# noir-lang/acvm

Hardware: AMD Instinct MI355X
Metric: witnesses solved/sec (whole node) (higher is better)
Workload: dtype u256 (8x u32 limbs, BN254-Fr Montgomery); 1 GPU; 10000-gate arithmetic-only ACIR, batch 2^20 witnesses over 1 GPU(s); opcodes=10000, global_batch=1048576, instances_per_gpu=1048576, tile_instances=131072, levels=41, not_solved_rank0_all_steps=68, algorithmic_bytes_per_witness=1025376, brillig_opcodes_inlined=0, parallelism=instances sharded x1, no collectives

## Files before the change

### acvm_amd/__init__.py

```python
import ctypes as C
import functools
import os

from . import acir

_HERE = os.path.dirname(os.path.abspath(__file__))
LIB_PATH = os.environ.get("ACVM_AMD_LIB") or os.path.join(_HERE, "libacvm_amd.so")

STATUS_SOLVED, STATUS_IN_PROGRESS, STATUS_FAILURE, STATUS_REQUIRES_FOREIGN_CALL = 0, 1, 2, 3
(ERR_NONE, ERR_MISSING_ASSIGNMENT, ERR_TOO_MANY_UNKNOWNS, ERR_UNSUPPORTED_BLACKBOX, ERR_UNSATISFIED, ERR_INDEX_OOB,
 ERR_BLACKBOX_FAILED, ERR_BRILLIG_FAILED, ERR_PANIC, ERR_DEVICE_LIMIT) = range(10)
LIMIT_BRILLIG_STEPS, LIMIT_BRILLIG_CALL_DEPTH, LIMIT_BRILLIG_MEMORY, LIMIT_DEVICE_MEMORY = 1, 2, 3, 4
ENC_BE32, ENC_LE32, ENC_MONT256_LE = 0, 1, 2
ENC_U8, ENC_U16, ENC_U32, ENC_U64, ENC_U128 = 16, 17, 18, 19, 20
LAYOUT_INSTANCE_MAJOR, LAYOUT_WITNESS_MAJOR = 0, 1
LAYOUT_BROADCAST = 16

ABI_SYMBOLS = [
    "acvm_last_error", "acvm_abi_version", "acvm_device_count", "acvm_set_device", "acvm_device_synchronize",
    "acvm_device_arch", "acvm_selftest", "acvm_debug_grumpkin", "acvm_debug_secp", "acvm_circuit_from_bytes", "acvm_circuit_free", "acvm_circuit_num_opcodes",
    "acvm_circuit_num_witnesses", "acvm_circuit_plan_stats", "acvm_batch_new", "acvm_batch_free", "acvm_batch_set_initial_witness",
    "acvm_batch_set_initial_witness_device", "acvm_batch_solve", "acvm_batch_solve_then_import", "acvm_batch_reset", "acvm_batch_set_instances", "acvm_batch_set_force_slow_path",
    "acvm_batch_results", "acvm_batch_witness", "acvm_batch_witness_map", "acvm_batch_stats",
    "acvm_batch_set_profiling", "acvm_batch_pending_foreign_call", "acvm_batch_pending_foreign_call_inputs",
    "acvm_batch_resolve_foreign_call", "acvm_circuit_assert_message", "acvm_circuit_witness_set", "acvm_batch_error_string",
    "acvm_batch_extract_witnesses", "acvm_batch_digest", "acvm_witness_map_decode", "acvm_witness_map_encode", "acvm_batch_witness_map_bytes",
    "acvm_device_malloc", "acvm_device_free", "acvm_device_upload", "acvm_batch_solve_opcode", "acvm_bb_stubbed", "acvm_bb_dummy",
    "acvm_new", "acvm_free", "acvm_solve", "acvm_solve_opcode", "acvm_get_status", "acvm_instruction_pointer", "acvm_witness_map", "acvm_finalize",
    "acvm_get_pending_foreign_call", "acvm_pending_foreign_call_inputs", "acvm_resolve_pending_foreign_call",
    "acvm_multi_new", "acvm_multi_free", "acvm_multi_num_groups", "acvm_multi_solve", "acvm_multi_results", "acvm_multi_num_witnesses",
    "acvm_multi_witness_map", "acvm_multi_locate", "acvm_debug_modmul_rate", "acvm_debug_secp_rate", "acvm_batch_new_ex", "acvm_circuit_plan_stats_ex",
    "acvm_tuning_set", "acvm_tuning_get", "acvm_tuning_key",
    "acvm_device_release_tables", "acvm_circuit_opcode_kinds", "acvm_batch_error_expression", "acvm_debug_stream_rate", "acvm_node_new", "acvm_node_free", "acvm_node_tile_instances", "acvm_node_num_devices", "acvm_node_solve", "acvm_node_stats",
    "acvm_debug_cpulist", "acvm_debug_device_locality", "acvm_debug_plan_fingerprint", "acvm_circuit_plans_built", "acvm_circuit_check_schedule", "acvm_batch_digest_blake2s",
    "acvm_batch_export_device", "acvm_device_download", "acvm_debug_fr", "acvm_debug_inverse_batch",
    "acvm_batch_import_device", "acvm_batch_solve_then_import_ex",
    "acvm_batch_import_device_parts", "acvm_debug_import_list_copies",
    "acvm_batch_import_device_masked", "acvm_batch_set_initial_witness_masked", "acvm_debug_import_missing",
    "acvm_debug_table_info", "acvm_debug_table_read", "acvm_debug_batch_tables",
    "acvm_batch_outcomes_device", "acvm_batch_export_device_list", "acvm_debug_export_h2d_bytes", "acvm_debug_select",
    "acvm_node_solve_device", "acvm_debug_node_io_bytes",
    "acvm_batch_foreign_call_sites", "acvm_batch_foreign_call_inputs_device", "acvm_batch_resolve_foreign_calls_device", "acvm_debug_foreign_call_stats",
    "acvm_batch_resolve_foreign_calls_device_rows",
    "acvm_node_set_foreign_call_handler", "acvm_node_foreign_stats",
    "acvm_batch_import_device_records", "acvm_batch_set_initial_witness_records", "acvm_node_solve_records",
    "acvm_batch_export_device_records", "acvm_batch_witness_records",
]


class AcvmError(RuntimeError):
    pass


class ExpressionHead(C.Structure):
    _fields_ = [("n_mul", C.c_uint32), ("n_lin", C.c_uint32), ("opcode_index", C.c_uint32), ("q_c", C.c_uint8 * 32)]


class ExportDesc(C.Structure):
# ... 364 lines not shown
    L.acvm_batch_results.argtypes = [C.c_void_p, C.c_void_p]
    L.acvm_batch_witness.argtypes = [C.c_void_p, C.c_uint32, C.c_void_p, C.c_void_p]
    L.acvm_batch_witness_map.argtypes = [C.c_void_p, C.c_uint32, C.c_uint32, C.c_void_p, C.c_void_p]
    L.acvm_batch_stats.argtypes = [C.c_void_p, C.POINTER(Stats)]
    L.acvm_batch_pending_foreign_call.argtypes = [C.c_void_p, C.c_uint32, C.POINTER(ForeignCallInfo)]
    L.acvm_batch_pending_foreign_call_inputs.argtypes = [C.c_void_p, C.c_uint32, C.c_void_p, C.c_void_p]
    L.acvm_batch_resolve_foreign_call.argtypes = [C.c_void_p, C.c_uint32, C.c_uint32, C.c_char_p, C.c_void_p, C.c_char_p]
    L.acvm_circuit_assert_message.argtypes = [C.c_void_p, C.c_uint32, C.c_uint32, C.c_char_p, C.c_size_t]
    L.acvm_circuit_witness_set.argtypes = [C.c_void_p, C.c_int, C.c_void_p, C.c_uint32]
    L.acvm_batch_error_string.argtypes = [C.c_void_p, C.c_void_p, C.c_uint32, C.c_char_p, C.c_size_t]
    L.acvm_batch_extract_witnesses.argtypes = [C.c_void_p, C.c_void_p, C.c_uint32, C.c_uint32, C.c_uint32, C.c_void_p]
    L.acvm_batch_digest.argtypes = [C.c_void_p, C.c_uint32, C.c_uint32, C.c_void_p]
    L.acvm_batch_digest_blake2s.argtypes = [C.c_void_p, C.c_uint32, C.c_uint32, C.c_void_p]
    for f in (L.acvm_witness_map_decode, L.acvm_witness_map_encode, L.acvm_batch_witness_map_bytes):
        f.restype = C.c_longlong
    L.acvm_witness_map_decode.argtypes = [C.c_char_p, C.c_size_t, C.c_void_p, C.c_void_p, C.c_uint32]
    L.acvm_witness_map_encode.argtypes = [C.c_void_p, C.c_char_p, C.c_uint32, C.c_void_p, C.c_size_t]
    L.acvm_batch_witness_map_bytes.argtypes = [C.c_void_p, C.c_uint32, C.c_void_p, C.c_size_t]
    L.acvm_debug_modmul_rate.argtypes = [C.c_uint32, C.c_uint32, C.POINTER(C.c_double), C.POINTER(C.c_uint64)]
    if hasattr(L, "acvm_debug_fr"):
        L.acvm_debug_fr.argtypes = [C.c_uint32, C.c_void_p, C.c_uint32, C.c_void_p, C.c_void_p]
        L.acvm_debug_inverse_batch.argtypes = [C.c_void_p, C.c_uint32, C.c_uint32, C.c_uint32, C.c_void_p, C.c_void_p, C.c_void_p, C.POINTER(C.c_uint32),
                                               C.POINTER(C.c_uint32)]
    L.acvm_debug_secp_rate.argtypes = [C.c_uint32, C.c_uint32, C.c_uint32, C.POINTER(C.c_double), C.POINTER(C.c_uint64)]
    L.acvm_circuit_opcode_kinds.argtypes = [C.c_void_p, C.c_uint32, C.c_uint32, C.c_void_p]
    L.acvm_batch_error_expression.argtypes = [C.c_void_p, C.c_void_p, C.c_uint32, C.POINTER(ExpressionHead), C.c_void_p, C.c_void_p, C.c_uint32, C.c_void_p, C.c_void_p, C.c_uint32]
    L.acvm_device_release_tables.restype = C.c_longlong
    L.acvm_device_release_tables.argtypes = [C.c_int]
    L.acvm_node_new.restype = C.c_void_p
    L.acvm_node_new.argtypes = [C.c_void_p, C.c_void_p, C.c_void_p, C.c_uint32, C.c_void_p, C.c_uint32, C.c_void_p]
    L.acvm_node_free.restype = None
    L.acvm_node_free.argtypes = [C.c_void_p]
    L.acvm_node_tile_instances.argtypes = [C.c_void_p]
    L.acvm_node_tile_instances.restype = C.c_uint32
    L.acvm_node_num_devices.argtypes = [C.c_void_p]
    L.acvm_node_num_devices.restype = C.c_uint32
    L.acvm_node_solve.restype = C.c_longlong
    L.acvm_node_solve.argtypes = [C.c_void_p, C.c_uint64, C.c_void_p, C.c_void_p, C.c_void_p, C.c_void_p, C.c_void_p]
    L.acvm_node_stats.argtypes = [C.c_void_p, C.c_void_p]
    L.acvm_debug_stream_rate.argtypes = [C.c_size_t, C.POINTER(C.c_double)]
    L.acvm_tuning_set.argtypes = [C.c_char_p, C.c_longlong]
    L.acvm_tuning_get.argtypes = [C.c_char_p, C.POINTER(C.c_longlong)]
    L.acvm_tuning_key.restype = C.c_char_p
    L.acvm_tuning_key.argtypes = [C.c_uint]
    L.acvm_device_malloc.restype = C.c_void_p
    L.acvm_device_malloc.argtypes = [C.c_size_t]
# ... 232 lines not shown
    assert all(len(it) == wi for it in items)
    data = b"".join(int(v).to_bytes(32, "big") for it in items for v in it)
    out = C.create_string_buffer(32 * wo * max(len(items), 1))
    _check(lib().acvm_debug_secp(curve, what, data, len(items), out))
    raw = out.raw
    return [tuple(int.from_bytes(raw[32 * (wo * i + k):32 * (wo * i + k + 1)], "big") for k in range(wo)) for i in range(len(items))]


FR_PROBE_WORDS = ((16, 8), (16, 8), (8, 8), (16, 8), (16, 8), (8, 8), (8, 8), (8, 8), (8, 8), (8, 2), (8, 2), (1, 8), (8, 9), (9, 8), (18, 9), (18, 9), (9, 9),
                  (9, 1), (9, 9), (10, 9), (9, 9), (9, 9), (9, 9), (9, 9), (19, 9), (18, 9), (9, 9), (9, 1), (18, 9), (36, 9), (54, 9), (27, 9), (45, 9), (27, 9),
                  (45, 9), (18, 9), (36, 9), (27, 9))


def debug_fr(what, items, uniform=None):
    import numpy as np
    wi, wo = FR_PROBE_WORDS[what]
    a = np.ascontiguousarray(items, dtype=np.uint32).reshape(-1, wi)
    out = np.zeros((a.shape[0], wo), dtype=np.uint32)
    u = None if uniform is None else np.ascontiguousarray(uniform, dtype=np.uint32).reshape(18)
    _check(lib().acvm_debug_fr(what, a.ctypes.data, a.shape[0], None if u is None else u.ctypes.data, out.ctypes.data))
    return out


def debug_inverse_batch(den, inv_chunk, slot_of=None):
    import numpy as np
    d = np.ascontiguousarray(den, dtype=np.uint32)
    n_jobs, B = d.shape[0], d.shape[1]
    assert d.shape == (n_jobs, B, 8)
    s = None if slot_of is None else np.ascontiguousarray(slot_of, dtype=np.uint32).reshape(n_jobs)
    inv, ev = np.zeros((n_jobs, B, 8), dtype=np.uint32), np.zeros(B, dtype=np.uint32)
    dc, hc = C.c_uint32(), C.c_uint32()
    _check(lib().acvm_debug_inverse_batch(d.ctypes.data, n_jobs, B, inv_chunk, None if s is None else s.ctypes.data, inv.ctypes.data, ev.ctypes.data,
                                          C.byref(dc), C.byref(hc)))
    return inv, ev, dc.value, hc.value


def debug_select(status, select_mask, out=None, want_list=True):
    import numpy as np
    st = np.ascontiguousarray(status, dtype=np.uint8).reshape(-1)
    n = st.shape[0]
    lst = None
    if want_list:
        lst = np.zeros(n, dtype=np.uint32) if out is None else np.ascontiguousarray(out, dtype=np.uint32).reshape(n).copy()
    count = C.c_uint32()
    _check(lib().acvm_debug_select(st.ctypes.data if n else None, n, select_mask, lst.ctypes.data if lst is not None and n else None, C.byref(count)))
    return lst, count.value


def decompress_witness(data: bytes) -> dict:
    n = _check(lib().acvm_witness_map_decode(data, len(data), None, None, 0))
    ids = (C.c_uint32 * max(n, 1))()
    vals = C.create_string_buffer(32 * max(n, 1))
    _check(lib().acvm_witness_map_decode(data, len(data), ids, vals, n))
    return {ids[i]: int.from_bytes(vals.raw[32 * i:32 * i + 32], "big") for i in range(n)}


# ... 722 lines not shown
```

### acvm_amd/csrc/batch_schedule.cpp

```cpp
#include <algorithm>
#include <chrono>
#include <cstdio>
#include <cstdlib>
#include <cstring>
#include <map>
#include <memory>
#include <new>
#include <stdexcept>
#include <string>
#include <vector>
#include "batch_internal.hpp"

struct LaunchTimers {
    std::vector<std::pair<hipEvent_t, hipEvent_t>> reg_pairs, dyn_pairs, cls_pairs[N_CLS];
    size_t ev_used = 0;
};

static int enqueue_level_schedule(acvm_batch *b, LaunchTimers *tm) {
    const Plan &p = b->plan();
    auto next_event = [&]() -> hipEvent_t {
        if (tm->ev_used == b->ev_pool.size()) {
            hipEvent_t e;
            hipEventCreate(&e);
            b->ev_pool.push_back(e);
// ... 19 lines not shown
            b->events_fresh = false;
            break;
        case SO_GATES:
            launch_arith_level(s, b->d_W, b->Bp, b->B, b->d_gate_stream, b->d_gate_offset + st.first, st.count, b->d_consts, b->d_event, b->d_inv);
            break;
        case SO_GATES_LIGHT:
            launch_arith_light_level(s, b->d_W, b->Bp, b->B, b->d_gate_stream, b->d_gate_offset + st.first, st.count, b->d_inv, b->dp,
                                     b->d_cls_offset[CLS_LIGHT] + st.first2, st.count2, b->d_event);
            break;
        case SO_LIGHT: launch_light_level(s, b->d_W, b->Bp, b->B, b->dp, off, st.count, b->d_event); break;
        case SO_LIGHT_SL: launch_light_sl_level(s, b->d_W, b->Bp, b->B, b->dp, off, st.count, b->d_event); break;
        case SO_HASH_COOP: launch_hash_coop_level(s, b->d_W, b->Bp, b->B, b->dp, off, st.count, b->d_event, st.lds_words); break;
        case SO_HASH: launch_hash_level(s, b->d_W, b->Bp, b->B, b->dp, off, soff, st.count, b->d_event, b->d_cls_scratch[k]); break;
        case SO_GRUMPKIN: launch_grumpkin_level(s, b->d_W, b->Bp, b->B, b->dp, off, soff, st.count, b->d_event, b->d_cls_scratch[k]); break;
        case SO_BRILLIG: launch_brillig_level(s, b->d_W, b->Bp, b->B, b->dp, off, soff, st.count, b->d_event, b->d_cls_scratch[k]); break;
        case SO_PEDERSEN: launch_pedersen_level(s, b->d_W, b->Bp, b->B, b->dp, off, st.count, b->d_event, soff, b->d_cls_scratch[k]); break;
        case SO_ECDSA: launch_ecdsa_level(s, b->d_W, b->Bp, b->B, b->dp, off, st.count, b->d_event); break;
        case SO_DIGEST: launch_digest_fold_level(s, b->d_W, b->Bp, b->B, b->dp, off, st.count, b->fp, b->d_leaves); break;
        case SO_HOSTBB:
            for (uint32_t r = 0; r < st.count; r++)
                if (int rc = run_host_blackbox(b, p.prog[p.cls_offset[k][st.first + r] + 1], false, 0)) return rc;
            break;
        case SO_INVERSE:
            launch_inverse_batch(s, b->d_W, b->d_inv, b->Bp, b->B, b->d_gate_stream, b->d_dyn_offset + st.first, st.count, b->d_event, (uint32_t)p.tune.inv_chunk);
            break;
        case SO_TRUNCATE: launch_event_truncate(s, b->d_event, b->B, p.truncated_at); break;
        }
        if (timed) {
            e1 = next_event();
            hipEventRecord(e1, s);
            (st.op == SO_GATES || st.op == SO_GATES_LIGHT ? tm->reg_pairs : st.op == SO_INVERSE ? tm->dyn_pairs : tm->cls_pairs[k]).push_back({e0, e1});
        }
        if (st.op == SO_GATES || st.op == SO_GATES_LIGHT) b->n_launches += (st.count + 65534) / 65535;
        else if (st.op != SO_EVENT_RESET && st.op != SO_TRUNCATE) b->n_launches++;
    }
    return 0;
}

static int ensure_level_events(acvm_batch *b) {
    const size_t n_levels = b->plan().n_levels;
    while (b->ev_sync.size() < 2 * n_levels + 1 || b->ev_heavy.size() < 4 * n_levels) {
        hipEvent_t e;
        HIPCHK(hipEventCreateWithFlags(&e, hipEventDisableTiming));
        (b->ev_sync.size() < 2 * n_levels + 1 ? b->ev_sync : b->ev_heavy).push_back(e);
    }
    return 0;
}
// ... 196 lines not shown
```

### acvm_amd/csrc/inverse_batch.hpp

```cpp
#pragma once
#include "fr_device.hpp"

namespace acvm {

template <class P>
FR_HD __forceinline__ void inverse_batch_body(const uint4 *__restrict__ W, uint4 *__restrict__ Inv, uint64_t Bp, uint64_t j, const uint32_t *__restrict__ gate_stream,
                                              const uint32_t *__restrict__ job_offset, uint32_t first, uint32_t n, uint32_t *__restrict__ event) {
    Fr29 prefix = fr29_from(fr_one());
    for (uint32_t i = 0; i < n; i++) {
        const uint32_t *__restrict__ g = gate_stream + job_offset[first + i];
        Fr den = P::load_den(W, g[0], Bp, j);
        if (fr_is_zero(den)) {
            P::flag(event, j, g[1]);
            den = fr_one();
        }
        prefix = fr29_mul(prefix, fr29_from(den));
        P::park(Inv, g[2], Bp, j, fr29_pack(prefix));
    }
    Fr29 inv = fr29_from(fr_inv(fr29_pack(fr29_cond_sub_p(prefix))));
    for (uint32_t i = n; i-- > 0;) {
        const uint32_t *__restrict__ g = gate_stream + job_offset[first + i];
        Fr den = P::load_den_last(W, g[0], Bp, j);
        if (fr_is_zero(den)) den = fr_one();
        const Fr prev = i > 0 ? P::parked(Inv, gate_stream[job_offset[first + i - 1] + 2], Bp, j) : fr_one();
        const Fr29 inv_i = fr29_mul(inv, fr29_from(prev));
        inv = fr29_mul(inv, fr29_from(den));
        P::store_inverse(Inv, g[2], Bp, j, fr29_pack(inv_i));
    }
}

}
```

### acvm_amd/csrc/kernels.hip

```cpp
#include "ops_common.hpp"
#include "fr_probe.hpp"
#include "inverse_batch.hpp"
#include "kernels.hpp"
#include "export_encode.hpp"
#include "export_source.hpp"
#include "tuning.hpp"

namespace acvm {

template <bool ALIGNED>
__global__ void __launch_bounds__(256) import_witness_kernel(uint4 *__restrict__ W, uint64_t Bp, uint32_t B,
                                                             const uint8_t *__restrict__ in, const uint32_t *__restrict__ ids,
                                                             uint32_t n_in, const uint32_t *__restrict__ gate, const uint32_t *__restrict__ plane_of_input,
                                                             uint32_t *__restrict__ plane, uint32_t *__restrict__ event_reset) {
    __shared__ uint4 tile[4][2][65];
    __shared__ uint32_t tile_low[4][64];
    if (gate && *gate != 0u) return;
    const uint32_t t = threadIdx.x;
    const uint64_t j0 = (uint64_t)blockIdx.x * 64u;
    const uint32_t k0 = blockIdx.y * 4u;
    {
        const uint32_t ji = t >> 2, kk = t & 3u;
        const uint64_t j = j0 + ji;
        const uint32_t k = k0 + kk;
// ... 262 lines not shown
__global__ void __launch_bounds__(ARITH_BLOCK) __attribute__((amdgpu_waves_per_eu(ARITH_WAVES_MIN, 8)))
arith_level_kernel(uint4 *__restrict__ W, uint64_t Bp, uint32_t B, const uint32_t *__restrict__ gate_stream, const uint32_t *__restrict__ gate_offset,
                   const uint32_t *__restrict__ consts, uint32_t *__restrict__ event, const uint4 *__restrict__ Inv) {
    arith_level_body(W, Bp, B, gate_stream, gate_offset, consts, event, Inv, blockIdx.y);
}

struct InverseDevicePolicy {
    static __device__ __forceinline__ Fr load_den(const uint4 *W, uint32_t row, uint64_t Bp, uint64_t j) { return fr_load(W, row, Bp, j); }
    static __device__ __forceinline__ Fr load_den_last(const uint4 *W, uint32_t row, uint64_t Bp, uint64_t j) { return fr_load_nt(W, row, Bp, j); }
    static __device__ __forceinline__ void park(uint4 *Inv, uint32_t slot, uint64_t Bp, uint64_t j, const Fr &a) { fr_store(Inv, slot, Bp, j, a); }
    static __device__ __forceinline__ Fr parked(const uint4 *Inv, uint32_t slot, uint64_t Bp, uint64_t j) { return fr_load(Inv, slot, Bp, j); }
    static __device__ __forceinline__ void store_inverse(uint4 *Inv, uint32_t slot, uint64_t Bp, uint64_t j, const Fr &a) { fr_store_nt(Inv, slot, Bp, j, a); }
    static __device__ __forceinline__ void flag(uint32_t *event, uint64_t j, uint32_t opcode) { flag_instance(event, j, opcode); }
};
__global__ void __launch_bounds__(64) inverse_batch_kernel(const uint4 *__restrict__ W, uint4 *__restrict__ Inv, uint64_t Bp, uint32_t B,
                                                           const uint32_t *__restrict__ gate_stream, const uint32_t *__restrict__ job_offset,
                                                           uint32_t n_jobs, uint32_t chunk, uint32_t *__restrict__ event) {
    const uint64_t j = (uint64_t)blockIdx.x * 64 + threadIdx.x;
    if (j >= B) return;
    const uint32_t first = blockIdx.y * chunk;
    const uint32_t n = n_jobs - first < chunk ? n_jobs - first : chunk;
    inverse_batch_body<InverseDevicePolicy>(W, Inv, Bp, j, gate_stream, job_offset, first, n, event);
}

__device__ __forceinline__ uint64_t st_mix(uint64_t &s) {
    s += 0x9E3779B97F4A7C15ULL;
    uint64_t z = s;
    z = (z ^ (z >> 30)) * 0xBF58476D1CE4E5B9ULL;
    z = (z ^ (z >> 27)) * 0x94D049BB133111EBULL;
    return z ^ (z >> 31);
}
__global__ void __launch_bounds__(256) fr_selftest_kernel(uint64_t seed, uint32_t n, uint32_t *mismatches) {
    const uint32_t i = blockIdx.x * blockDim.x + threadIdx.x;
    if (i >= n) return;
    uint64_t s = seed + 0x1234567ULL * i;
    Fr a, b;
    for (int k = 0; k < 4; k++) {
        uint64_t x = st_mix(s), y = st_mix(s);
        a.v[2 * k] = (uint32_t)x; a.v[2 * k + 1] = (uint32_t)(x >> 32);
        b.v[2 * k] = (uint32_t)y; b.v[2 * k + 1] = (uint32_t)(y >> 32);
    }
    a.v[7] &= 0x1fffffffu;
    b.v[7] &= 0x1fffffffu;
    if (i == 0) a = fr_zero();
    if (i == 1) { a = fr_modulus(); a.v[0] -= 1; }
    if (i == 2) b = fr_one();
// ... 224 lines not shown
    if (!n_lanes || !x.n_sel) return;
    const ExportArgs a{W, Bp, x.first, x.n, x.sel, x.n_sel, x.n_witnesses, nullptr, nullptr, nullptr, nullptr, x.encoding, x.stride, (uint4 *)x.out, x.mask};
    for (uint32_t done = 0; done < x.n_sel; done += 65535u) {
        const uint32_t m = x.n_sel - done > 65535u ? 65535u : x.n_sel - done;
        hipLaunchKernelGGL(export_device_lanes_kernel, dim3((n_lanes + 255u) / 256u, m), dim3(256), 0, s, a, lanes, n_lanes, side, assigned_bits, n_slow, x.layout, done);
    }
}
void launch_unscale_slow(hipStream_t s, uint4 *W, uint64_t Bp, const uint32_t *slow_ids, uint32_t n_slow, const Unscale &u, const uint32_t *producer,
                         const uint32_t *start_opcode) {
    const uint64_t n = (uint64_t)n_slow * u.n_scaled;
    if (!n) return;
    hipLaunchKernelGGL(unscale_slow_kernel, dim3((unsigned)((n + 255) / 256)), dim3(256), 0, s, W, Bp, slow_ids, n_slow, u.scaled_ids, u.n_scaled,
                       u.consts, producer, start_opcode);
}
void launch_arith_level(hipStream_t s, uint4 *W, uint64_t Bp, uint32_t B, const uint32_t *gate_stream, const uint32_t *gate_offset,
                        uint32_t n_gates, const uint32_t *consts, uint32_t *event, const uint4 *inv) {
    for (uint32_t done = 0; done < n_gates;) {
        uint32_t n = n_gates - done > 65535u ? 65535u : n_gates - done;
        hipLaunchKernelGGL(arith_level_kernel, dim3((B + ARITH_BLOCK - 1) / ARITH_BLOCK, n), dim3(ARITH_BLOCK), 0, s, W, Bp, B, gate_stream, gate_offset + done, consts, event, inv);
        done += n;
    }
}
void launch_inverse_batch(hipStream_t s, const uint4 *W, uint4 *inv, uint64_t Bp, uint32_t B, const uint32_t *gate_stream,
                          const uint32_t *job_offset, uint32_t n_jobs, uint32_t *event, uint32_t inv_chunk) {
    if (!n_jobs || !B) return;
    const uint32_t cap = std::min<uint32_t>(std::max<uint32_t>(inv_chunk, 1), 65536), n_chunks = (n_jobs + cap - 1) / cap;
    const uint32_t chunk = (n_jobs + n_chunks - 1) / n_chunks;
    for (uint32_t done = 0; done < n_jobs;) {
        const uint32_t n = (uint32_t)std::min<uint64_t>(n_jobs - done, (uint64_t)chunk * 65535u);
        hipLaunchKernelGGL(inverse_batch_kernel, dim3((B + 63) / 64, (n + chunk - 1) / chunk), dim3(64), 0, s, W, inv, Bp, B, gate_stream, job_offset + done, n, chunk, event);
        done += n;
    }
}
void launch_fr_selftest(hipStream_t s, uint64_t seed, uint32_t n, uint32_t *mismatches) {
    if (!n) return;
    hipLaunchKernelGGL(fr_selftest_kernel, dim3((n + 255) / 256), dim3(256), 0, s, seed, n, mismatches);
}
__global__ void __launch_bounds__(256) event_reset_kernel(uint32_t *__restrict__ event, uint32_t B) {
    const uint32_t i = blockIdx.x * 256 + threadIdx.x;
    if (i < B) event[i] = 0xFFFFFFFFu;
    else if (i < B + 2) event[(int)(i - B) - 4] = 0u;
}
__global__ void __launch_bounds__(256) event_truncate_kernel(uint32_t *__restrict__ event, uint32_t B, uint32_t opcode) {
    const uint32_t i = blockIdx.x * 256 + threadIdx.x;
    if (i < B) event[i] = min(event[i], opcode);
    if (i == 0) event[-4] = B;
}
void launch_event_reset(hipStream_t s, uint32_t *event, uint32_t B) {
    hipLaunchKernelGGL(event_reset_kernel, dim3((B + 2) / 256 + 1), dim3(256), 0, s, event, B);
}
void launch_event_truncate(hipStream_t s, uint32_t *event, uint32_t B, uint32_t opcode) {
    if (B) hipLaunchKernelGGL(event_truncate_kernel, dim3((B + 255) / 256), dim3(256), 0, s, event, B, opcode);
}
// ... 18 lines not shown
```

### acvm_amd/csrc/kernels.hpp

```cpp
#pragma once
#include "grumpkin_host.hpp"
#include <hip/hip_runtime.h>
#include <stdint.h>

namespace acvm {

struct SlowResult {
    uint32_t status, err, opcode_index, aux0, aux1;
    uint32_t msg, x0, x1;
    uint32_t n_call_stack;
    uint32_t call_stack[16];
    uint32_t val[8];
};

struct FcStoreSlot {
    const uint32_t *desc;
    const uint4 *vals;
};
struct FcLanes {
    uint32_t *pend_desc;
    uint32_t pend_desc_words;
    uint4 *pend_vals;
    uint32_t pend_vals_cap;
};
// ... 109 lines not shown
    uint32_t n_witnesses;
    const uint32_t *row_of, *producer;
    const uint32_t *u_index, *u_plain, *u_m256;
    uint8_t *out;
    uint64_t pitch;
    const uint32_t *windows, *fields;
};
void launch_export_records(hipStream_t s, const RecordExport &x, uint32_t n_windows);
void launch_outcomes_fill(hipStream_t s, uint32_t n, uint8_t *status, uint8_t *err, uint32_t *opcode_index);
void launch_outcomes_lanes(hipStream_t s, const uint32_t *records, uint32_t n_lanes, uint32_t n, uint8_t *status, uint8_t *err, uint32_t *opcode_index);
void launch_lane_map_scatter(hipStream_t s, int32_t *lane_of, uint32_t n_instances, const uint32_t *ids, uint32_t n_slow);
void launch_scatter_rows32(hipStream_t s, const uint32_t *rows, const uint32_t *lanes, uint32_t n_lanes, uint32_t n, uint8_t *out);
size_t select_scratch_words(uint32_t n);
void launch_select(hipStream_t s, const uint8_t *status, uint32_t first, uint32_t n, uint32_t select_mask, uint32_t *scratch, uint32_t *out, uint32_t *count);
void launch_gather_initial(hipStream_t s, uint4 *Wx, uint64_t Bpx, const uint4 *W, uint64_t Bp, const uint32_t *init_ids, const uint32_t *init_rows, uint32_t n_init,
                           const uint32_t *slow_ids, uint32_t n_slow);
void launch_gather_columns(hipStream_t s, uint4 *Wx, uint64_t Bpx, const uint4 *W, uint64_t Bp, uint32_t n_rows, const uint32_t *slow_ids, uint32_t n_slow,
                           const uint32_t *unscale_index, const uint32_t *unscale_consts, const uint32_t *producer, const uint32_t *start_opcode);
void launch_unscale_slow(hipStream_t s, uint4 *W, uint64_t Bp, const uint32_t *slow_ids, uint32_t n_slow, const Unscale &u, const uint32_t *producer,
                         const uint32_t *start_opcode);
void launch_arith_level(hipStream_t s, uint4 *W, uint64_t Bp, uint32_t B, const uint32_t *gate_stream, const uint32_t *gate_offset,
                        uint32_t n_gates, const uint32_t *consts, uint32_t *event, const uint4 *inv);
void launch_inverse_batch(hipStream_t s, const uint4 *W, uint4 *inv, uint64_t Bp, uint32_t B, const uint32_t *gate_stream,
                          const uint32_t *job_offset, uint32_t n_jobs, uint32_t *event, uint32_t inv_chunk);
void launch_arith_light_level(hipStream_t s, uint4 *W, uint64_t Bp, uint32_t B, const uint32_t *gate_stream, const uint32_t *gate_offset, uint32_t n_gates,
                              const uint4 *inv, const DeviceProgram &dp, const uint32_t *light_offsets, uint32_t n_light, uint32_t *event);
void launch_modmul_rate(hipStream_t s, uint32_t *out, uint32_t blocks, uint32_t iters);
void launch_secp_rate(hipStream_t s, uint32_t curve, uint32_t *out, uint32_t blocks, uint32_t iters);
void launch_stream_rate(hipStream_t s, const uint4 *a, const uint4 *b, uint4 *out, uint64_t n);
void launch_fr_selftest(hipStream_t s, uint64_t seed, uint32_t n, uint32_t *mismatches);
uint32_t fr_probe_words(uint32_t what, bool out);
void launch_fr_probe(hipStream_t s, uint32_t what, const uint32_t *in, uint32_t n_items, const uint32_t *uniform18, uint32_t *out);
void launch_fill_u32(hipStream_t s, uint32_t *p, uint32_t v, uint64_t n);
void launch_event_reset(hipStream_t s, uint32_t *event, uint32_t B);
void launch_event_truncate(hipStream_t s, uint32_t *event, uint32_t B, uint32_t opcode);
void launch_min_u32(hipStream_t s, uint32_t *p, uint32_t v, uint64_t n);
void launch_init_assigned(hipStream_t s, uint32_t *assigned, uint32_t n_slow, uint32_t n_words, uint32_t n_witnesses,
                          const uint32_t *producer, const uint32_t *start_opcode);

void launch_light_level(hipStream_t s, uint4 *W, uint64_t Bp, uint32_t B, const DeviceProgram &dp, const uint32_t *offsets, uint32_t n,
                        uint32_t *event);
void launch_light_sl_level(hipStream_t s, uint4 *W, uint64_t Bp, uint32_t B, const DeviceProgram &dp, const uint32_t *offsets, uint32_t n,
                           uint32_t *event);
void launch_hash_level(hipStream_t s, uint4 *W, uint64_t Bp, uint32_t B, const DeviceProgram &dp, const uint32_t *offsets,
                       const uint32_t *scratch_off, uint32_t n, uint32_t *event, uint32_t *scratch);
void launch_hash_coop_level(hipStream_t s, uint4 *W, uint64_t Bp, uint32_t B, const DeviceProgram &dp, const uint32_t *offsets, uint32_t n, uint32_t *event, uint32_t lds_words);
void launch_grumpkin_level(hipStream_t s, uint4 *W, uint64_t Bp, uint32_t B, const DeviceProgram &dp, const uint32_t *offsets,
// ... 75 lines not shown
```

### acvm_amd/csrc/probes.cpp

```cpp
#include <algorithm>
#include <chrono>
#include <cstdio>
#include <cstdlib>
#include <cstring>
#include <map>
#include <memory>
#include <new>
#include <stdexcept>
#include <string>
#include <vector>
#include "batch_internal.hpp"

int acvm_selftest(uint32_t n, uint64_t seed) {
    uint32_t *d = nullptr, h = 0;
    HIPCHK(hipMalloc((void **)&d, 4));
    HIPCHK(hipMemset(d, 0, 4));
    launch_fr_selftest(nullptr, seed, n, d);
    HIPCHK(hipGetLastError());
    HIPCHK(hipDeviceSynchronize());
    HIPCHK(hipMemcpy(&h, d, 4, hipMemcpyDeviceToHost));
    hipFree(d);
    return (int)h;
}

// ... 199 lines not shown
    const uint32_t wi = fr_probe_words(what, false), wo = fr_probe_words(what, true);
    if (!wi || !wo) return set_err(ACVM_E_INVALID, "no such routine");
    if (!n_items) return 0;
    if (!in || !out) return set_err(ACVM_E_INVALID, "null argument");
    uint32_t *d_in = nullptr, *d_out = nullptr;
    HIPCHK(hipMalloc((void **)&d_in, (size_t)n_items * wi * 4));
    if (hipMalloc((void **)&d_out, (size_t)n_items * wo * 4) != hipSuccess) {
        hipFree(d_in);
        return set_err(ACVM_E_DEVICE, "hipMalloc failed");
    }
    int rc = 0;
    auto step = [&](hipError_t e, const char *what_) { if (!rc && e != hipSuccess) rc = set_err(ACVM_E_DEVICE, std::string(what_) + ": " + hipGetErrorString(e)); };
    step(hipMemcpy(d_in, in, (size_t)n_items * wi * 4, hipMemcpyHostToDevice), "hipMemcpy");
    step(hipMemset(d_out, 0, (size_t)n_items * wo * 4), "hipMemset");
    if (!rc) launch_fr_probe(nullptr, what, d_in, n_items, uniform18, d_out);
    step(hipGetLastError(), "fr_probe_kernel");
    step(hipDeviceSynchronize(), "hipDeviceSynchronize");
    step(hipMemcpy(out, d_out, (size_t)n_items * wo * 4, hipMemcpyDeviceToHost), "hipMemcpy");
    hipFree(d_in);
    hipFree(d_out);
    return rc;
} ABI_CATCH

int acvm_debug_inverse_batch(const uint32_t *den, uint32_t n_jobs, uint32_t B, uint32_t inv_chunk, const uint32_t *slot_of, uint32_t *inv_out,
                             uint32_t *event_out, uint32_t *device_count, uint32_t *host_count) try {
    if (!den || !n_jobs || !B || !inv_out || !event_out || !device_count || !host_count) return set_err(ACVM_E_INVALID, "bad argument");
    if (slot_of) {
        std::vector<uint8_t> seen(n_jobs, 0);
        for (uint32_t k = 0; k < n_jobs; k++) {
            if (slot_of[k] >= n_jobs || seen[slot_of[k]]) return set_err(ACVM_E_INVALID, "slot_of is not a permutation");
            seen[slot_of[k]] = 1;
        }
    }
    const uint64_t Bp = ((uint64_t)B + 63) / 64 * 64;
    const size_t row = (size_t)2 * Bp, table_bytes = (size_t)n_jobs * row * sizeof(uint4);
    std::vector<uint4> hW((size_t)n_jobs * row, make_uint4(0, 0, 0, 0));
    std::vector<uint32_t> stream((size_t)n_jobs * 3), offset(n_jobs);
    for (uint32_t k = 0; k < n_jobs; k++) {
        for (uint32_t j = 0; j < B; j++) {
            const uint32_t *v = den + ((size_t)k * B + j) * 8;
            hW[(size_t)k * row + j] = make_uint4(v[0], v[1], v[2], v[3]);
            hW[(size_t)k * row + Bp + j] = make_uint4(v[4], v[5], v[6], v[7]);
        }
        stream[3 * (size_t)k] = k;
        stream[3 * (size_t)k + 1] = k;
        stream[3 * (size_t)k + 2] = slot_of ? slot_of[k] : k;
        offset[k] = 3 * k;
    }
    struct Mem {
        uint4 *W = nullptr, *inv = nullptr;
        uint32_t *stream = nullptr, *offset = nullptr, *event_base = nullptr, *event = nullptr, *h_count = nullptr;
        ~Mem() {
            for (void *p : {(void *)W, (void *)inv, (void *)stream, (void *)offset, (void *)event_base})
                if (p) hipFree(p);
            if (h_count) hipHostFree(h_count);
        }
    } m;
    HIPCHK(hipMalloc((void **)&m.W, table_bytes));
    HIPCHK(hipMalloc((void **)&m.inv, table_bytes));
    HIPCHK(hipMemcpy(m.W, hW.data(), table_bytes, hipMemcpyHostToDevice));
    HIPCHK(hipMemset(m.inv, 0, table_bytes));
    if (int rc = upload(&m.stream, stream)) return rc;
    if (int rc = upload(&m.offset, offset)) return rc;
    if (int rc = event_words_new(B, &m.event_base, &m.event, &m.h_count)) return rc;
    *m.h_count = 0;
    launch_event_reset(nullptr, m.event, B);
    launch_inverse_batch(nullptr, m.W, m.inv, Bp, B, m.stream, m.offset, n_jobs, m.event, inv_chunk);
    HIPCHK(hipGetLastError());
    HIPCHK(hipDeviceSynchronize());
    HIPCHK(hipMemcpy(hW.data(), m.inv, table_bytes, hipMemcpyDeviceToHost));
    HIPCHK(hipMemcpy(event_out, m.event, (size_t)B * 4, hipMemcpyDeviceToHost));
    HIPCHK(hipMemcpy(device_count, m.event - 4, 4, hipMemcpyDeviceToHost));
    *host_count = *(volatile uint32_t *)m.h_count;
    for (uint32_t k = 0; k < n_jobs; k++)
        for (uint32_t j = 0; j < B; j++) {
            const uint4 lo = hW[(size_t)k * row + j], hi = hW[(size_t)k * row + Bp + j];
            uint32_t *v = inv_out + ((size_t)k * B + j) * 8;
            v[0] = lo.x; v[1] = lo.y; v[2] = lo.z; v[3] = lo.w; v[4] = hi.x; v[5] = hi.y; v[6] = hi.z; v[7] = hi.w;
        }
    return 0;
} ABI_CATCH

int acvm_debug_select(const uint8_t *status, uint32_t n, uint32_t select_mask, uint32_t *out_list, uint32_t *n_selected) try {
    if (!n_selected || (n && !status)) return set_err(ACVM_E_INVALID, "null argument");
    struct Mem {
        uint8_t *status = nullptr;
        uint32_t *list = nullptr, *scratch = nullptr;
        ~Mem() {
            for (void *p : {(void *)status, (void *)list, (void *)scratch})
                if (p) hipFree(p);
        }
    } m;
    const size_t words = select_scratch_words(n);
    HIPCHK(hipMalloc((void **)&m.status, n ? n : 1));
    HIPCHK(hipMalloc((void **)&m.scratch, (words + 1) * 4));
    if (n) HIPCHK(hipMemcpy(m.status, status, n, hipMemcpyHostToDevice));
    if (out_list && n) {
        HIPCHK(hipMalloc((void **)&m.list, (size_t)n * 4));
        HIPCHK(hipMemcpy(m.list, out_list, (size_t)n * 4, hipMemcpyHostToDevice));
    }
    launch_select(nullptr, m.status, 0, n, select_mask, m.scratch, m.list, m.scratch + words);
    HIPCHK(hipGetLastError());
    HIPCHK(hipDeviceSynchronize());
// ... 5 lines not shown
```

### acvm_amd/csrc/tuning.cpp

```cpp
#include "tuning.hpp"
#include <cstdlib>
#include <cstring>
#include <mutex>
#include <string>

namespace acvm {
namespace {

struct Key { const char *name; int64_t Tuning::*field; };
const Key KEYS[] = {
    {"scale", &Tuning::scale}, {"relax", &Tuning::relax}, {"pedersen_bundle", &Tuning::pedersen_bundle}, {"pedersen_bundle_waves", &Tuning::pedersen_bundle_waves}, {"pairs", &Tuning::pairs}, {"chains", &Tuning::chains}, {"max_tails", &Tuning::max_tails},
    {"inv_epoch", &Tuning::inv_epoch}, {"inv_latency", &Tuning::inv_latency}, {"inv_chunk", &Tuning::inv_chunk}, {"byte_plane", &Tuning::byte_plane}, {"heavy_epoch", &Tuning::heavy_epoch}, {"heavy_latency", &Tuning::heavy_latency},
    {"pedersen_latency", &Tuning::pedersen_latency}, {"pedersen_epoch", &Tuning::pedersen_epoch}, {"digest_epoch", &Tuning::digest_epoch}, {"range_fuse", &Tuning::range_fuse},
    {"range_merge", &Tuning::range_merge}, {"hash_chain", &Tuning::hash_chain}, {"brillig_inline", &Tuning::brillig_inline}, {"sl_lane", &Tuning::sl_lane},
    {"pedersen_waves", &Tuning::pedersen_waves}, {"pedersen_prio", &Tuning::pedersen_prio}, {"light_fuse", &Tuning::light_fuse}, {"plan_validate", &Tuning::plan_validate}, {"brillig_mem_cells", &Tuning::brillig_mem_cells}, {"overlap", &Tuning::overlap}, {"heavy_streams", &Tuning::heavy_streams}, {"heavy_only_streams", &Tuning::heavy_only_streams},
    {"fc_relevel", &Tuning::fc_relevel}, {"exact_async", &Tuning::exact_async}, {"brillig_steps_log2", &Tuning::brillig_steps_log2},
    {"brillig_steps_max_log2", &Tuning::brillig_steps_max_log2}, {"brillig_call_depth", &Tuning::brillig_call_depth},
    {"brillig_call_depth_max", &Tuning::brillig_call_depth_max}, {"brillig_mem_max_log2", &Tuning::brillig_mem_max_log2},
    {"pedersen_window_bits", &Tuning::pedersen_window_bits}, {"win16", &Tuning::win16}, {"tables_keep", &Tuning::tables_keep},
};
constexpr unsigned N_KEYS = sizeof KEYS / sizeof KEYS[0];

Tuning g_tuning;
std::once_flag g_env_once;

void read_env() {
    const char *e = getenv("ACVM_TUNING");
    if (!e) return;
    std::string s(e);
    size_t at = 0;
    while (at < s.size()) {
        size_t end = s.find(',', at);
        if (end == std::string::npos) end = s.size();
        const std::string item = s.substr(at, end - at);
        const size_t eq = item.find('=');
// ... 34 lines not shown
```

### acvm_amd/csrc/tuning.hpp

```cpp
#pragma once
#include <stdint.h>

namespace acvm {

struct Tuning {
    int64_t scale = 1;
    int64_t relax = 1;
    int64_t pairs = 1;
    int64_t chains = 1;
    int64_t max_tails = 5;
    int64_t inv_epoch = 4;
    int64_t byte_plane = 1;
    int64_t inv_chunk = 128;
    int64_t inv_latency = 1;
    int64_t heavy_epoch = 1;
    int64_t heavy_latency = 0;
    int64_t pedersen_latency = 4;
    int64_t pedersen_epoch = 8;
    int64_t digest_epoch = 8;
    int64_t range_fuse = 1;
    int64_t range_merge = 1;
    int64_t hash_chain = 1;
    int64_t brillig_inline = 1;
    int64_t sl_lane = 0;
    int64_t pedersen_waves = 0;
    int64_t pedersen_bundle = 1;
    int64_t pedersen_bundle_waves = 2048;
    int64_t pedersen_prio = 1;
    int64_t light_fuse = 1;
    int64_t plan_validate = 0;
    int64_t brillig_mem_cells = 0;
    int64_t overlap = 1;
    int64_t heavy_streams = 1;
    int64_t heavy_only_streams = 1;
    int64_t fc_relevel = -1;
    int64_t exact_async = 1;
// ... 15 lines not shown
```

### include/acvm_amd.h

```cpp
#ifndef ACVM_AMD_H
#define ACVM_AMD_H
#include <stddef.h>
#include <stdint.h>

#ifdef __cplusplus
extern "C" {
#endif

#define ACVM_AMD_ABI_VERSION 6

enum {
    ACVM_OK = 0,
    ACVM_E_INVALID = -1,
    ACVM_E_MALFORMED = -2,
    ACVM_E_UNSUPPORTED = -3,
    ACVM_E_DEVICE = -4,
    ACVM_E_STATE = -5,
    ACVM_E_NOMEM = -6
};

enum { ACVM_STATUS_SOLVED = 0, ACVM_STATUS_IN_PROGRESS = 1, ACVM_STATUS_FAILURE = 2, ACVM_STATUS_REQUIRES_FOREIGN_CALL = 3 };

enum {
    ACVM_ERR_NONE = 0,
// ... 73 lines not shown

const char *acvm_last_error(void);
int acvm_abi_version(void);
int acvm_device_count(void);
int acvm_set_device(int device);
int acvm_device_synchronize(void);
int acvm_device_arch(char *out, size_t out_len);
long long acvm_device_release_tables(int device);

int acvm_tuning_set(const char *key, long long value);
int acvm_tuning_get(const char *key, long long *value);
const char *acvm_tuning_key(unsigned index);

int acvm_selftest(uint32_t n, uint64_t seed);

int acvm_debug_grumpkin(uint32_t what, uint32_t param, const uint8_t *in_be32, uint32_t n_in, uint8_t *out_be64);
int acvm_debug_table_info(uint32_t table, uint64_t *n_entries, int *built);
int acvm_debug_table_read(uint32_t table, const uint64_t *entries, uint32_t n, uint32_t *out_words16);
int acvm_debug_batch_tables(const acvm_batch_t *b, uint32_t *mask);
int acvm_debug_secp(uint32_t curve, uint32_t what, const uint8_t *in_be32, uint32_t n_items, uint8_t *out_be32);
int acvm_debug_fr(uint32_t what, const uint32_t *in, uint32_t n_items, const uint32_t *uniform18, uint32_t *out);
int acvm_debug_inverse_batch(const uint32_t *den, uint32_t n_jobs, uint32_t B, uint32_t inv_chunk, const uint32_t *slot_of, uint32_t *inv_out,
                             uint32_t *event_out, uint32_t *device_count, uint32_t *host_count);
int acvm_debug_select(const uint8_t *status, uint32_t n, uint32_t select_mask, uint32_t *out_list, uint32_t *n_selected);

int acvm_debug_modmul_rate(uint32_t iters, uint32_t waves_per_simd, double *modmul_per_s, uint64_t *n_modmul);
int acvm_debug_secp_rate(uint32_t curve, uint32_t iters, uint32_t waves_per_simd, double *products_per_s, uint64_t *n_products);
int acvm_debug_stream_rate(size_t bytes, double *gb_per_s);

acvm_circuit_t *acvm_circuit_from_bytes(const uint8_t *bytes, size_t len);
void acvm_circuit_free(acvm_circuit_t *c);
uint32_t acvm_circuit_num_opcodes(const acvm_circuit_t *c);
uint32_t acvm_circuit_num_witnesses(const acvm_circuit_t *c);
int acvm_circuit_opcode_kinds(const acvm_circuit_t *c, uint32_t first, uint32_t n, uint32_t *kinds );
int acvm_circuit_plan_stats(const acvm_circuit_t *c, const uint32_t *initial_ids, uint32_t n_initial, acvm_stats_t *out);
uint64_t acvm_circuit_plans_built(const acvm_circuit_t *c);
int acvm_circuit_plan_stats_ex(const acvm_circuit_t *c, const uint32_t *initial_ids, uint32_t n_initial, uint32_t flags, const uint32_t *keep_ids,
                               uint32_t n_keep, acvm_stats_t *out);

int acvm_circuit_check_schedule(const acvm_circuit_t *c, const uint32_t *initial_ids, uint32_t n_initial, uint32_t flags, const uint32_t *keep_ids, uint32_t n_keep,
                                uint32_t n_instances, uint32_t drop_wait, uint64_t *counts , char *report, size_t report_len);
int acvm_debug_plan_fingerprint(const acvm_circuit_t *c, const uint32_t *initial_ids, uint32_t n_initial, uint32_t flags, const uint32_t *keep_ids,
                                uint32_t n_keep, uint64_t *out, uint32_t cap);
acvm_batch_t *acvm_batch_new(const acvm_circuit_t *c, const acvm_bb_solver_t *solver, uint32_t n_instances,
                             const uint32_t *initial_ids, uint32_t n_initial);
#define ACVM_BATCH_FOLD_DIGEST 1u
// ... 299 lines not shown
```

Baseline: 6.041 million witnesses/s.

## Share one field inversion across waves in batch-inverse kernel

Adds a shared-memory variant of the batched inverse kernel where G waves (default 4) in a workgroup pool their prefix-product totals, one wave computes a single field inversion of the product, and each wave recovers its own inverse by multiplying with the other waves' totals. This is Montgomery's trick applied across waves, so the number of expensive modular inversions per chunk drops by a factor of G. In exchange it adds extra multiplications, LDS traffic, two block barriers, and serializes the inversion onto one wave while the others wait. A new inv_share tuning key selects G, and a debug entry point exposes it.

```diff
diff --git a/acvm_amd/__init__.py b/acvm_amd/__init__.py
--- a/acvm_amd/__init__.py
+++ b/acvm_amd/__init__.py
@@ -33,7 +33,7 @@
     "acvm_tuning_set", "acvm_tuning_get", "acvm_tuning_key",
     "acvm_device_release_tables", "acvm_circuit_opcode_kinds", "acvm_batch_error_expression", "acvm_debug_stream_rate", "acvm_node_new", "acvm_node_free", "acvm_node_tile_instances", "acvm_node_num_devices", "acvm_node_solve", "acvm_node_stats",
     "acvm_debug_cpulist", "acvm_debug_device_locality", "acvm_debug_plan_fingerprint", "acvm_circuit_plans_built", "acvm_circuit_check_schedule", "acvm_batch_digest_blake2s",
-    "acvm_batch_export_device", "acvm_device_download", "acvm_debug_fr", "acvm_debug_inverse_batch",
+    "acvm_batch_export_device", "acvm_device_download", "acvm_debug_fr", "acvm_debug_inverse_batch", "acvm_debug_inverse_batch_shared",
     "acvm_batch_import_device", "acvm_batch_solve_then_import_ex",
     "acvm_batch_import_device_parts", "acvm_debug_import_list_copies",
     "acvm_batch_import_device_masked", "acvm_batch_set_initial_witness_masked", "acvm_debug_import_missing",
@@ -444,6 +444,9 @@
         L.acvm_debug_fr.argtypes = [C.c_uint32, C.c_void_p, C.c_uint32, C.c_void_p, C.c_void_p]
         L.acvm_debug_inverse_batch.argtypes = [C.c_void_p, C.c_uint32, C.c_uint32, C.c_uint32, C.c_void_p, C.c_void_p, C.c_void_p, C.POINTER(C.c_uint32),
                                                C.POINTER(C.c_uint32)]
+    if hasattr(L, "acvm_debug_inverse_batch_shared"):
+        L.acvm_debug_inverse_batch_shared.argtypes = [C.c_void_p, C.c_uint32, C.c_uint32, C.c_uint32, C.c_uint32, C.c_void_p, C.c_void_p, C.c_void_p,
+                                                      C.POINTER(C.c_uint32), C.POINTER(C.c_uint32)]
     L.acvm_debug_secp_rate.argtypes = [C.c_uint32, C.c_uint32, C.c_uint32, C.POINTER(C.c_double), C.POINTER(C.c_uint64)]
     L.acvm_circuit_opcode_kinds.argtypes = [C.c_void_p, C.c_uint32, C.c_uint32, C.c_void_p]
     L.acvm_batch_error_expression.argtypes = [C.c_void_p, C.c_void_p, C.c_uint32, C.POINTER(ExpressionHead), C.c_void_p, C.c_void_p, C.c_uint32, C.c_void_p, C.c_void_p, C.c_uint32]
@@ -722,7 +725,7 @@
     return out
 
 
-def debug_inverse_batch(den, inv_chunk, slot_of=None):
+def debug_inverse_batch(den, inv_chunk, slot_of=None, inv_share=None):
     import numpy as np
     d = np.ascontiguousarray(den, dtype=np.uint32)
     n_jobs, B = d.shape[0], d.shape[1]
@@ -730,8 +733,12 @@
     s = None if slot_of is None else np.ascontiguousarray(slot_of, dtype=np.uint32).reshape(n_jobs)
     inv, ev = np.zeros((n_jobs, B, 8), dtype=np.uint32), np.zeros(B, dtype=np.uint32)
     dc, hc = C.c_uint32(), C.c_uint32()
-    _check(lib().acvm_debug_inverse_batch(d.ctypes.data, n_jobs, B, inv_chunk, None if s is None else s.ctypes.data, inv.ctypes.data, ev.ctypes.data,
-                                          C.byref(dc), C.byref(hc)))
+    if inv_share is None:
+        _check(lib().acvm_debug_inverse_batch(d.ctypes.data, n_jobs, B, inv_chunk, None if s is None else s.ctypes.data, inv.ctypes.data, ev.ctypes.data,
+                                              C.byref(dc), C.byref(hc)))
+    else:
+        _check(lib().acvm_debug_inverse_batch_shared(d.ctypes.data, n_jobs, B, inv_chunk, inv_share, None if s is None else s.ctypes.data, inv.ctypes.data,
+                                                     ev.ctypes.data, C.byref(dc), C.byref(hc)))
     return inv, ev, dc.value, hc.value
 
 
diff --git a/acvm_amd/csrc/batch_schedule.cpp b/acvm_amd/csrc/batch_schedule.cpp
--- a/acvm_amd/csrc/batch_schedule.cpp
+++ b/acvm_amd/csrc/batch_schedule.cpp
@@ -65,7 +65,8 @@
                 if (int rc = run_host_blackbox(b, p.prog[p.cls_offset[k][st.first + r] + 1], false, 0)) return rc;
             break;
         case SO_INVERSE:
-            launch_inverse_batch(s, b->d_W, b->d_inv, b->Bp, b->B, b->d_gate_stream, b->d_dyn_offset + st.first, st.count, b->d_event, (uint32_t)p.tune.inv_chunk);
+            launch_inverse_batch(s, b->d_W, b->d_inv, b->Bp, b->B, b->d_gate_stream, b->d_dyn_offset + st.first, st.count, b->d_event, (uint32_t)p.tune.inv_chunk,
+                                 inverse_share_clamp(p.tune.inv_share));
             break;
         case SO_TRUNCATE: launch_event_truncate(s, b->d_event, b->B, p.truncated_at); break;
         }
diff --git a/acvm_amd/csrc/inverse_batch.hpp b/acvm_amd/csrc/inverse_batch.hpp
--- a/acvm_amd/csrc/inverse_batch.hpp
+++ b/acvm_amd/csrc/inverse_batch.hpp
@@ -4,8 +4,8 @@
 namespace acvm {
 
 template <class P>
-FR_HD __forceinline__ void inverse_batch_body(const uint4 *__restrict__ W, uint4 *__restrict__ Inv, uint64_t Bp, uint64_t j, const uint32_t *__restrict__ gate_stream,
-                                              const uint32_t *__restrict__ job_offset, uint32_t first, uint32_t n, uint32_t *__restrict__ event) {
+FR_HD __forceinline__ Fr29 inverse_batch_forward(const uint4 *__restrict__ W, uint4 *__restrict__ Inv, uint64_t Bp, uint64_t j, const uint32_t *__restrict__ gate_stream,
+                                                 const uint32_t *__restrict__ job_offset, uint32_t first, uint32_t n, uint32_t *__restrict__ event) {
     Fr29 prefix = fr29_from(fr_one());
     for (uint32_t i = 0; i < n; i++) {
         const uint32_t *__restrict__ g = gate_stream + job_offset[first + i];
@@ -17,7 +17,12 @@
         prefix = fr29_mul(prefix, fr29_from(den));
         P::park(Inv, g[2], Bp, j, fr29_pack(prefix));
     }
-    Fr29 inv = fr29_from(fr_inv(fr29_pack(fr29_cond_sub_p(prefix))));
+    return prefix;
+}
+
+template <class P>
+FR_HD __forceinline__ void inverse_batch_backward(const uint4 *__restrict__ W, uint4 *__restrict__ Inv, uint64_t Bp, uint64_t j, const uint32_t *__restrict__ gate_stream,
+                                                  const uint32_t *__restrict__ job_offset, uint32_t first, uint32_t n, Fr29 inv) {
     for (uint32_t i = n; i-- > 0;) {
         const uint32_t *__restrict__ g = gate_stream + job_offset[first + i];
         Fr den = P::load_den_last(W, g[0], Bp, j);
@@ -29,4 +34,49 @@
     }
 }
 
+template <int G, class Totals>
+FR_HD __forceinline__ Fr29 inverse_share_total_inverse(const Totals &totals) {
+    Fr29 t = totals(0);
+#pragma unroll 1
+    for (uint32_t v = 1; v < (uint32_t)G; v++) t = fr29_mul(t, totals(v));
+    return fr29_from(fr_inv(fr29_pack(fr29_cond_sub_p(t))));
 }
+template <int G, class Totals>
+FR_HD __forceinline__ Fr29 inverse_share_own(const Totals &totals, const Fr29 &inv_all, uint32_t w) {
+    if constexpr (G == 1) {
+        return inv_all;
+    } else {
+        Fr29 s = inv_all;
+#pragma unroll 1
+        for (uint32_t v = 0; v < (uint32_t)G; v++)
+            if (v != w) s = fr29_mul(s, totals(v));
+        return fr29_cond_sub_p(s);
+    }
+}
+constexpr uint32_t INVERSE_SHARE_ROW_WORDS = 9 * 64;
+FR_HD __forceinline__ void inverse_share_row_store(uint32_t *rows, uint32_t row, uint32_t lane, const Fr29 &a) {
+#pragma unroll
+    for (int i = 0; i < 9; i++) rows[row * INVERSE_SHARE_ROW_WORDS + i * 64 + lane] = a.v[i];
+}
+FR_HD __forceinline__ Fr29 inverse_share_row_load(const uint32_t *rows, uint32_t row, uint32_t lane) {
+    Fr29 r;
+#pragma unroll
+    for (int i = 0; i < 9; i++) r.v[i] = rows[row * INVERSE_SHARE_ROW_WORDS + i * 64 + lane];
+    return r;
+}
+struct InverseShareRows {
+    const uint32_t *rows;
+    uint32_t lane;
+    FR_HD __forceinline__ Fr29 operator()(uint32_t v) const { return inverse_share_row_load(rows, v, lane); }
+};
+
+template <class P>
+FR_HD __forceinline__ void inverse_batch_body(const uint4 *__restrict__ W, uint4 *__restrict__ Inv, uint64_t Bp, uint64_t j, const uint32_t *__restrict__ gate_stream,
+                                              const uint32_t *__restrict__ job_offset, uint32_t first, uint32_t n, uint32_t *__restrict__ event) {
+    const Fr29 total = inverse_batch_forward<P>(W, Inv, Bp, j, gate_stream, job_offset, first, n, event);
+    const auto totals = [&](uint32_t) { return total; };
+    const Fr29 inv = inverse_share_total_inverse<1>(totals);
+    inverse_batch_backward<P>(W, Inv, Bp, j, gate_stream, job_offset, first, n, inverse_share_own<1>(totals, inv, 0));
+}
+
+}
diff --git a/acvm_amd/csrc/kernels.hip b/acvm_amd/csrc/kernels.hip
--- a/acvm_amd/csrc/kernels.hip
+++ b/acvm_amd/csrc/kernels.hip
@@ -308,6 +308,27 @@
     const uint32_t n = n_jobs - first < chunk ? n_jobs - first : chunk;
     inverse_batch_body<InverseDevicePolicy>(W, Inv, Bp, j, gate_stream, job_offset, first, n, event);
 }
+template <int G>
+__global__ void __launch_bounds__(64 * G) inverse_batch_kernel_shared(const uint4 *__restrict__ W, uint4 *__restrict__ Inv, uint64_t Bp, uint32_t B,
+                                                                      const uint32_t *__restrict__ gate_stream, const uint32_t *__restrict__ job_offset,
+                                                                      uint32_t n_jobs, uint32_t chunk, uint32_t *__restrict__ event) {
+    __shared__ uint32_t rows[(G + 1) * INVERSE_SHARE_ROW_WORDS];
+    const uint32_t lane = threadIdx.x & 63u, w = __builtin_amdgcn_readfirstlane(threadIdx.x >> 6);
+    const uint64_t j = (uint64_t)blockIdx.x * (64 * G) + threadIdx.x;
+    const bool live = j < B;
+    const uint32_t first = blockIdx.y * chunk;
+    const uint32_t n = n_jobs - first < chunk ? n_jobs - first : chunk;
+    Fr29 total = fr29_from(fr_one());
+    if (live) total = inverse_batch_forward<InverseDevicePolicy>(W, Inv, Bp, j, gate_stream, job_offset, first, n, event);
+    inverse_share_row_store(rows, w, lane, total);
+    __syncthreads();
+    const InverseShareRows totals{rows, lane};
+    if (w == 0) inverse_share_row_store(rows, G, lane, inverse_share_total_inverse<G>(totals));
+    __syncthreads();
+    if (live)
+        inverse_batch_backward<InverseDevicePolicy>(W, Inv, Bp, j, gate_stream, job_offset, first, n,
+                                                    inverse_share_own<G>(totals, inverse_share_row_load(rows, G, lane), w));
+}
 
 __device__ __forceinline__ uint64_t st_mix(uint64_t &s) {
     s += 0x9E3779B97F4A7C15ULL;
@@ -578,13 +599,15 @@
     }
 }
 void launch_inverse_batch(hipStream_t s, const uint4 *W, uint4 *inv, uint64_t Bp, uint32_t B, const uint32_t *gate_stream,
-                          const uint32_t *job_offset, uint32_t n_jobs, uint32_t *event, uint32_t inv_chunk) {
+                          const uint32_t *job_offset, uint32_t n_jobs, uint32_t *event, uint32_t inv_chunk, uint32_t inv_share) {
     if (!n_jobs || !B) return;
+    const uint32_t G = inverse_share_clamp(inv_share), waves = (B + 63) / 64;
+    const auto kernel = G == 8 ? inverse_batch_kernel_shared<8> : G == 4 ? inverse_batch_kernel_shared<4> : G == 2 ? inverse_batch_kernel_shared<2> : inverse_batch_kernel;
     const uint32_t cap = std::min<uint32_t>(std::max<uint32_t>(inv_chunk, 1), 65536), n_chunks = (n_jobs + cap - 1) / cap;
     const uint32_t chunk = (n_jobs + n_chunks - 1) / n_chunks;
     for (uint32_t done = 0; done < n_jobs;) {
         const uint32_t n = (uint32_t)std::min<uint64_t>(n_jobs - done, (uint64_t)chunk * 65535u);
-        hipLaunchKernelGGL(inverse_batch_kernel, dim3((B + 63) / 64, (n + chunk - 1) / chunk), dim3(64), 0, s, W, inv, Bp, B, gate_stream, job_offset + done, n, chunk, event);
+        hipLaunchKernelGGL(kernel, dim3((waves + G - 1) / G, (n + chunk - 1) / chunk), dim3(64 * G), 0, s, W, inv, Bp, B, gate_stream, job_offset + done, n, chunk, event);
         done += n;
     }
 }
diff --git a/acvm_amd/csrc/kernels.hpp b/acvm_amd/csrc/kernels.hpp
--- a/acvm_amd/csrc/kernels.hpp
+++ b/acvm_amd/csrc/kernels.hpp
@@ -155,7 +155,8 @@
 void launch_arith_level(hipStream_t s, uint4 *W, uint64_t Bp, uint32_t B, const uint32_t *gate_stream, const uint32_t *gate_offset,
                         uint32_t n_gates, const uint32_t *consts, uint32_t *event, const uint4 *inv);
 void launch_inverse_batch(hipStream_t s, const uint4 *W, uint4 *inv, uint64_t Bp, uint32_t B, const uint32_t *gate_stream,
-                          const uint32_t *job_offset, uint32_t n_jobs, uint32_t *event, uint32_t inv_chunk);
+                          const uint32_t *job_offset, uint32_t n_jobs, uint32_t *event, uint32_t inv_chunk, uint32_t inv_share);
+inline uint32_t inverse_share_clamp(int64_t v) { return v >= 8 ? 8u : v >= 4 ? 4u : v >= 2 ? 2u : 1u; }
 void launch_arith_light_level(hipStream_t s, uint4 *W, uint64_t Bp, uint32_t B, const uint32_t *gate_stream, const uint32_t *gate_offset, uint32_t n_gates,
                               const uint4 *inv, const DeviceProgram &dp, const uint32_t *light_offsets, uint32_t n_light, uint32_t *event);
 void launch_modmul_rate(hipStream_t s, uint32_t *out, uint32_t blocks, uint32_t iters);
diff --git a/acvm_amd/csrc/probes.cpp b/acvm_amd/csrc/probes.cpp
--- a/acvm_amd/csrc/probes.cpp
+++ b/acvm_amd/csrc/probes.cpp
@@ -245,8 +245,8 @@
     return rc;
 } ABI_CATCH
 
-int acvm_debug_inverse_batch(const uint32_t *den, uint32_t n_jobs, uint32_t B, uint32_t inv_chunk, const uint32_t *slot_of, uint32_t *inv_out,
-                             uint32_t *event_out, uint32_t *device_count, uint32_t *host_count) try {
+static int debug_inverse_batch(const uint32_t *den, uint32_t n_jobs, uint32_t B, uint32_t inv_chunk, uint32_t inv_share, const uint32_t *slot_of, uint32_t *inv_out,
+                               uint32_t *event_out, uint32_t *device_count, uint32_t *host_count) {
     if (!den || !n_jobs || !B || !inv_out || !event_out || !device_count || !host_count) return set_err(ACVM_E_INVALID, "bad argument");
     if (slot_of) {
         std::vector<uint8_t> seen(n_jobs, 0);
@@ -288,7 +288,7 @@
     if (int rc = event_words_new(B, &m.event_base, &m.event, &m.h_count)) return rc;
     *m.h_count = 0;
     launch_event_reset(nullptr, m.event, B);
-    launch_inverse_batch(nullptr, m.W, m.inv, Bp, B, m.stream, m.offset, n_jobs, m.event, inv_chunk);
+    launch_inverse_batch(nullptr, m.W, m.inv, Bp, B, m.stream, m.offset, n_jobs, m.event, inv_chunk, inv_share);
     HIPCHK(hipGetLastError());
     HIPCHK(hipDeviceSynchronize());
     HIPCHK(hipMemcpy(hW.data(), m.inv, table_bytes, hipMemcpyDeviceToHost));
@@ -302,6 +302,14 @@
             v[0] = lo.x; v[1] = lo.y; v[2] = lo.z; v[3] = lo.w; v[4] = hi.x; v[5] = hi.y; v[6] = hi.z; v[7] = hi.w;
         }
     return 0;
+}
+int acvm_debug_inverse_batch(const uint32_t *den, uint32_t n_jobs, uint32_t B, uint32_t inv_chunk, const uint32_t *slot_of, uint32_t *inv_out,
+                             uint32_t *event_out, uint32_t *device_count, uint32_t *host_count) try {
+    return debug_inverse_batch(den, n_jobs, B, inv_chunk, inverse_share_clamp(tuning().inv_share), slot_of, inv_out, event_out, device_count, host_count);
+} ABI_CATCH
+int acvm_debug_inverse_batch_shared(const uint32_t *den, uint32_t n_jobs, uint32_t B, uint32_t inv_chunk, uint32_t inv_share, const uint32_t *slot_of,
+                                    uint32_t *inv_out, uint32_t *event_out, uint32_t *device_count, uint32_t *host_count) try {
+    return debug_inverse_batch(den, n_jobs, B, inv_chunk, inverse_share_clamp(inv_share), slot_of, inv_out, event_out, device_count, host_count);
 } ABI_CATCH
 
 int acvm_debug_select(const uint8_t *status, uint32_t n, uint32_t select_mask, uint32_t *out_list, uint32_t *n_selected) try {
diff --git a/acvm_amd/csrc/tuning.cpp b/acvm_amd/csrc/tuning.cpp
--- a/acvm_amd/csrc/tuning.cpp
+++ b/acvm_amd/csrc/tuning.cpp
@@ -10,7 +10,7 @@
 struct Key { const char *name; int64_t Tuning::*field; };
 const Key KEYS[] = {
     {"scale", &Tuning::scale}, {"relax", &Tuning::relax}, {"pedersen_bundle", &Tuning::pedersen_bundle}, {"pedersen_bundle_waves", &Tuning::pedersen_bundle_waves}, {"pairs", &Tuning::pairs}, {"chains", &Tuning::chains}, {"max_tails", &Tuning::max_tails},
-    {"inv_epoch", &Tuning::inv_epoch}, {"inv_latency", &Tuning::inv_latency}, {"inv_chunk", &Tuning::inv_chunk}, {"byte_plane", &Tuning::byte_plane}, {"heavy_epoch", &Tuning::heavy_epoch}, {"heavy_latency", &Tuning::heavy_latency},
+    {"inv_epoch", &Tuning::inv_epoch}, {"inv_latency", &Tuning::inv_latency}, {"inv_chunk", &Tuning::inv_chunk}, {"inv_share", &Tuning::inv_share}, {"byte_plane", &Tuning::byte_plane}, {"heavy_epoch", &Tuning::heavy_epoch}, {"heavy_latency", &Tuning::heavy_latency},
     {"pedersen_latency", &Tuning::pedersen_latency}, {"pedersen_epoch", &Tuning::pedersen_epoch}, {"digest_epoch", &Tuning::digest_epoch}, {"range_fuse", &Tuning::range_fuse},
     {"range_merge", &Tuning::range_merge}, {"hash_chain", &Tuning::hash_chain}, {"brillig_inline", &Tuning::brillig_inline}, {"sl_lane", &Tuning::sl_lane},
     {"pedersen_waves", &Tuning::pedersen_waves}, {"pedersen_prio", &Tuning::pedersen_prio}, {"light_fuse", &Tuning::light_fuse}, {"plan_validate", &Tuning::plan_validate}, {"brillig_mem_cells", &Tuning::brillig_mem_cells}, {"overlap", &Tuning::overlap}, {"heavy_streams", &Tuning::heavy_streams}, {"heavy_only_streams", &Tuning::heavy_only_streams},
diff --git a/acvm_amd/csrc/tuning.hpp b/acvm_amd/csrc/tuning.hpp
--- a/acvm_amd/csrc/tuning.hpp
+++ b/acvm_amd/csrc/tuning.hpp
@@ -12,6 +12,7 @@
     int64_t inv_epoch = 4;
     int64_t byte_plane = 1;
     int64_t inv_chunk = 128;
+    int64_t inv_share = 4;
     int64_t inv_latency = 1;
     int64_t heavy_epoch = 1;
     int64_t heavy_latency = 0;
diff --git a/include/acvm_amd.h b/include/acvm_amd.h
--- a/include/acvm_amd.h
+++ b/include/acvm_amd.h
@@ -119,6 +119,8 @@
 int acvm_debug_fr(uint32_t what, const uint32_t *in, uint32_t n_items, const uint32_t *uniform18, uint32_t *out);
 int acvm_debug_inverse_batch(const uint32_t *den, uint32_t n_jobs, uint32_t B, uint32_t inv_chunk, const uint32_t *slot_of, uint32_t *inv_out,
                              uint32_t *event_out, uint32_t *device_count, uint32_t *host_count);
+int acvm_debug_inverse_batch_shared(const uint32_t *den, uint32_t n_jobs, uint32_t B, uint32_t inv_chunk, uint32_t inv_share, const uint32_t *slot_of,
+                                    uint32_t *inv_out, uint32_t *event_out, uint32_t *device_count, uint32_t *host_count);
 int acvm_debug_select(const uint8_t *status, uint32_t n, uint32_t select_mask, uint32_t *out_list, uint32_t *n_selected);
 
 int acvm_debug_modmul_rate(uint32_t iters, uint32_t waves_per_simd, double *modmul_per_s, uint64_t *n_modmul);
```

New measurement: 6.157 million witnesses/s (median of 6 runs). 1.9% higher.
